# lightkurve/lightkurve

Hardware: NVIDIA B200
Metric: lombscargle_freqbins_x_cadences_per_s (higher is better)
Workload: dtype f32 spreading + FFT, f64 phase (nufft)

## Files before the change

### lightkurve_b200/csrc/nufft_v2.cuh

```cuda
#pragma once
#include "nufft_core.h"

namespace lkb {
namespace {

using nufft::V2_PB;
using nufft::V2_THREADS;
using nufft::V2_TILE;
constexpr int V2_LOG_TILE = 13;
static_assert((1 << V2_LOG_TILE) == V2_TILE, "tile size");
constexpr int V2_BC = 1 << V2_PB;
constexpr int V2_R = V2_TILE / (2 * V2_BC);
constexpr int V2_LSB = V2_BC + V2_BC / 16 + 1;
constexpr int V2R_P_MIN = V2_PB + 4 + 1, V2R_P_MAX = V2_PB + 13 + 1;

__host__ __device__ constexpr int v2_radix(int plog, int idx) {
  return (idx < plog / 4) ? 16 : ((idx == plog / 4 && (plog % 4)) ? (1 << (plog % 4)) : 0);
}
__host__ __device__ constexpr int v2_log2i(int r) { return r == 16 ? 4 : r == 8 ? 3 : r == 4 ? 2 : r == 2 ? 1 : 0; }
__device__ __forceinline__ int v2_skew(int a) { return a + (a >> 4); }
template <int nb>
__host__ __device__ constexpr int v2_in_off(int r) {
  return (nb % 16 == 0) ? r * (nb + nb / 16) : r * nb + ((r * nb) >> 4);
}

template <class CT>
__global__ void nufft2_tables_kernel(int pa, int pb, int ph, CT* __restrict__ tw_a, CT* __restrict__ tw_b,
                                     CT* __restrict__ t_hi, CT* __restrict__ t_lo) {
  const int la = nufft::v2_pass_table_len(pa), lb = nufft::v2_pass_table_len(pb), pl = nufft::v2_log2_lo(ph);
  const int nlo = 1 << pl, nhi = 1 << (ph - pl);
  int e = (int)(blockIdx.x * blockDim.x + threadIdx.x);
  int64_t num = 0, den = 1;
  CT* dst = nullptr;
  if (e < la) { nufft::v2_pass_table_entry(pa, e, &num, &den); dst = tw_a + e; }
  else if ((e -= la) < lb) { nufft::v2_pass_table_entry(pb, e, &num, &den); dst = tw_b + e; }
  else if ((e -= lb) < nhi) { num = e; den = nhi; dst = t_hi + e; }
  else if ((e -= nhi) < nlo) { num = e; den = (int64_t)1 << ph; dst = t_lo + e; }
  else return;
  double sn, cs;
  sincospi(2.0 * (double)num / (double)den, &sn, &cs);
  typedef typename nufft::CplxOf<CT>::real RT;
  *dst = nufft::CplxOf<CT>::mk((RT)cs, (RT)sn);
}

template <class RT>
__global__ void nufft2_weights_kernel(const double* __restrict__ t, int64_t N, double df, int64_t M, int w, double beta,
                                      RT* __restrict__ Wt) {
  const int64_t e = (int64_t)blockIdx.x * blockDim.x + threadIdx.x;
  if (e >= N * w) return;
  const int64_t n = e / w;
  const int q = (int)(e - n * w);
  const double x = df * t[n] * (double)M + (double)nufft::grid_shift(w);
  const double i0 = ceil(x - 0.5 * (double)w);
  const double z = (i0 + (double)q - x) * (2.0 / (double)w);
  const double s2 = 1.0 - z * z;
  Wt[e] = (s2 > 0.0) ? (RT)exp(beta * (sqrt(s2) - 1.0)) : (RT)0.0;
}

__device__ __forceinline__ int64_t v2_zcell_of(int64_t e, int ptc, int n1max) {
  const int64_t j = e & (((int64_t)1 << ptc) - 1), rest = e >> ptc;
  const int64_t n1 = rest % n1max, c = rest / n1max;
  return (n1 << V2_PB) + (c << ptc) + j;
}

template <int LCS>
__global__ void __launch_bounds__(256)
nufft2_spread_kernel(const int32_t* __restrict__ first_ge, const nufft::Cad* __restrict__ cad,
                     const float* __restrict__ Wt, const float* __restrict__ y, int64_t ystride, int B, int w, int p,
                     int ptc, int n1max, float2* __restrict__ G) {
  const int64_t cells = (int64_t)n1max << V2_PB;
  const int64_t e = (int64_t)blockIdx.x * blockDim.x + threadIdx.x;
  if (e >= cells) return;
  const int64_t M = (int64_t)1 << p, m = 2 * v2_zcell_of(e, ptc, n1max);
  const int lc0 = (int)blockIdx.y * LCS;
  const float* yr[LCS];
#pragma unroll
  for (int q = 0; q < LCS; ++q) {
    int b = lc0 + q;
    if (b > B - 1) b = B - 1;
    yr[q] = y + (int64_t)b * ystride;
  }
  float a0[LCS], a1[LCS];
#pragma unroll
  for (int q = 0; q < LCS; ++q) { a0[q] = 0.0f; a1[q] = 0.0f; }
  const int64_t L = nufft::table_len(M, w);
  for (int wrap = 0; wrap < 2; ++wrap) {
    const int64_t mm = m + (int64_t)wrap * M;
    if (mm + 1 >= L) break;
    int64_t lo_c = mm - w + 1, hi_c = mm + 2;
    if (lo_c < 0) lo_c = 0;
    if (hi_c > L - 1) hi_c = L - 1;
    const int32_t na = first_ge[lo_c], nb = first_ge[hi_c];
    for (int32_t n = na; n < nb; ++n) {
      const int tap = (int)(mm - (int64_t)cad[n].i0);
      const float* wr = Wt + (int64_t)n * w;
      const float w0 = (tap >= 0) ? wr[tap] : 0.0f;
      const float w1 = (tap + 1 < w) ? wr[tap + 1] : 0.0f;
#pragma unroll
      for (int q = 0; q < LCS; ++q) {
        const float v = yr[q][n];
        a0[q] = fmaf(w0, v, a0[q]);
        a1[q] = fmaf(w1, v, a1[q]);
      }
    }
  }
#pragma unroll
  for (int q = 0; q < LCS; ++q)
    if (lc0 + q < B) G[(int64_t)(lc0 + q) * cells + e] = make_float2(a0[q], a1[q]);
}

template <int PLOG, int LS, int IDX, int NS, class CT = float2>
__device__ __forceinline__ void v2_pass_t(CT* buf, const CT* __restrict__ tw, int nz = 1 << 30) {
  constexpr int R = v2_radix(PLOG, IDX);
  if constexpr (R != 0) {
    constexpr int LR = v2_log2i(R), NB = 16 / R, PNB = PLOG - LR, nb = 1 << PNB;
    constexpr bool WIDE = nb > V2_THREADS;
    static_assert(WIDE || (V2_THREADS % nb) == 0, "geometry");
    const int t = (int)threadIdx.x;
    CT u[NB][R];
    int base_in[NB];
#pragma unroll
    for (int q = 0; q < NB; ++q) {
      int line, i;
      if constexpr (WIDE) { line = 0; i = t + V2_THREADS * q; }
      else { line = (t >> PNB) + ((V2_THREADS * q) >> PNB); i = t & (nb - 1); }
      base_in[q] = line * LS + ((nb % 16 == 0) ? v2_skew(i) : i);
#pragma unroll
      for (int r = 0; r < R; ++r)
        u[q][r] = (IDX > 0 || r * nb < nz) ? buf[base_in[q] + v2_in_off<nb>(r)] : nufft::CplxOf<CT>::mk(0, 0);
    }
    __syncthreads();
#pragma unroll
    for (int q = 0; q < NB; ++q) {
      int line, i;
      if constexpr (WIDE) { line = 0; i = t + V2_THREADS * q; }
      else { line = (t >> PNB) + ((V2_THREADS * q) >> PNB); i = t & (nb - 1); }
      const int k = i & (NS - 1);
      if constexpr (NS > 1) {
#pragma unroll
        for (int r = 1; r < R; ++r) u[q][r] = nufft::cmul(u[q][r], tw[r * NS + k]);
      }
      nufft::SmallDft<R, CT>::run(u[q]);
      const int j = ((i - k) << LR) + k;
      const int base_out = line * LS + ((NS == 1) ? (j + i) : v2_skew(j));
#pragma unroll
      for (int r = 0; r < R; ++r) buf[base_out + ((NS == 1) ? r : r * (NS + NS / 16))] = u[q][r];
    }
    __syncthreads();
    v2_pass_t<PLOG, LS, IDX + 1, NS * R, CT>(buf, tw + ((IDX > 0) ? R * NS : 0));
  }
}

struct V2Count {
  const int* count;
  int base, cap;
};
__device__ __forceinline__ int v2_count(const V2Count nc, int grid_y) {
  if (!nc.count) return grid_y;
  const int n = *nc.count - nc.base;
  return n < 0 ? 0 : (n > nc.cap ? nc.cap : n);
}

template <int PA, class CT>
__device__ __forceinline__ void v2_cols_one(CT* buf, const CT* __restrict__ G, CT* __restrict__ T, int n1max,
                                            const CT* __restrict__ tw_a, const CT* __restrict__ t_hi,
                                            const CT* __restrict__ t_lo, const int64_t lc) {
  constexpr int A = 1 << PA, PTC = V2_LOG_TILE - PA, TC = 1 << PTC, LS = A + A / 16 + 1, C = V2_BC / TC;
  constexpr int JW = TC < 32 ? TC : 32, RW = V2_THREADS / JW, CG = TC / JW;
  constexpr int LJW = JW == 32 ? 5 : JW == 16 ? 4 : JW == 8 ? 3 : JW == 4 ? 2 : JW == 2 ? 1 : 0;
  static_assert((1 << LJW) == JW && RW % 16 == 0, "geometry");
  const int t = (int)threadIdx.x, c = (int)blockIdx.x;
  const int jl = t & (JW - 1), nl = t >> LJW;
  const int nvalid = n1max << PTC;
  const CT* Gp = G + (lc * C + c) * (int64_t)nvalid;
  const int s_base = jl * LS + v2_skew(nl), g_base = nl * TC + jl;
  constexpr int NB1 = A / v2_radix(PA, 0);
  const int nz = ((n1max + NB1 - 1) / NB1) * NB1;
#pragma unroll
  for (int u = 0; u < 16; ++u) {
    const int cg = u % CG, nbk = u / CG;
    if (nbk * RW < nz) {
      const int idx = g_base + nbk * RW * TC + cg * JW;
      buf[s_base + cg * JW * LS + nbk * (RW + RW / 16)] = (idx < nvalid) ? Gp[idx] : nufft::CplxOf<CT>::mk(0, 0);
    }
  }
  __syncthreads();
  v2_pass_t<PA, LS, 0, 1, CT>(buf, tw_a, nz);
  CT* Tp = T + (lc * C + c) * (int64_t)V2_TILE;
  const int ph = PA + V2_PB, pl = nufft::v2_log2_lo(ph);
  const unsigned Mmask = (1u << ph) - 1u, lmask = (1u << pl) - 1u;
#pragma unroll
  for (int u = 0; u < 16; ++u) {
    const int cg = u % CG, nbk = u / CG;
    const int k1 = nl + nbk * RW, n2 = c * TC + jl + cg * JW;
    const unsigned q = ((unsigned)n2 * (unsigned)k1) & Mmask;
    const CT wq = nufft::cmul(t_hi[q >> pl], t_lo[q & lmask]);
    Tp[g_base + nbk * RW * TC + cg * JW] = nufft::cmul(buf[s_base + cg * JW * LS + nbk * (RW + RW / 16)], wq);
  }
}
template <int PA, class CT = float2>
__global__ void __launch_bounds__(V2_THREADS, sizeof(CT) == 8 ? 2 : 1)
nufft2_cols_kernel(const CT* __restrict__ G, CT* __restrict__ T, int n1max, const CT* __restrict__ tw_a,
                   const CT* __restrict__ t_hi, const CT* __restrict__ t_lo) {
  LKB_DYN_SMEM(CT, buf);
  v2_cols_one<PA, CT>(buf, G, T, n1max, tw_a, t_hi, t_lo, (int64_t)blockIdx.y);
}
template <int PA>
__global__ void __launch_bounds__(V2_THREADS, 1)
nufft2_cols_list_kernel(const double2* __restrict__ G, double2* __restrict__ T, int n1max,
                        const double2* __restrict__ tw_a, const double2* __restrict__ t_hi,
                        const double2* __restrict__ t_lo, V2Count nc) {
  LKB_DYN_SMEM(double2, buf);
  const int64_t ntr = v2_count(nc, (int)gridDim.y);
  for (int64_t lc = blockIdx.y; lc < ntr; lc += gridDim.y) {
    __syncthreads();
    v2_cols_one<PA, double2>(buf, G, T, n1max, tw_a, t_hi, t_lo, lc);
  }
}

struct V2FTab {
  float4 d;
  float4 c;
};
struct V2Finish {
  const V2FTab* ftab;
  int64_t k0, F, k_lo;
  const float* ysum;
  float Nf;
  int normalization;
  float scale;
  float* power;
  unsigned* peak;
  const int* lcmap;
  int log2M;
};

__device__ __forceinline__ float v2_normalise(float pw, float Nf, int normalization, float scale) {
  if (normalization == LKB_LS_NORM_PSD_SCALE) return pw * scale;
  if (normalization == LKB_LS_NORM_AMPLITUDE) return sqrtf(pw * (4.0f / Nf));
  return pw;
}
__device__ __forceinline__ float v2_finish_pw(float2 g1, float2 g2, const V2FTab tb, float ysum, int64_t, int) {
  const float ex = 0.5f * (g1.x + g2.x), ey = 0.5f * (g1.y - g2.y);
  const float ox = 0.5f * (g1.y + g2.y), oy = 0.5f * (g2.x - g1.x);
  const float yc = ex * tb.d.x - ey * tb.d.y + ox * tb.d.z - oy * tb.d.w - ysum * tb.c.x;
  const float ys = ex * tb.d.y + ey * tb.d.x + ox * tb.d.w + oy * tb.d.z - ysum * tb.c.y;
  return yc * yc * tb.c.z + ys * ys * tb.c.w;
}
__device__ __forceinline__ float v2_finish_pw(double2 g1, double2 g2, const V2FTab tb, float ysum, int64_t kk, int log2M) {
  const double ex = 0.5 * (g1.x + g2.x), ey = 0.5 * (g1.y - g2.y);
  const double ox = 0.5 * (g1.y + g2.y), oy = 0.5 * (g2.x - g1.x);
  double sw, cw;
  sincospi(ldexp((double)kk, 1 - log2M), &sw, &cw);
  const double gx = ex + cw * ox - sw * oy, gy = ey + cw * oy + sw * ox;
  const double yc = gx * (double)tb.d.x - gy * (double)tb.d.y - (double)ysum * (double)tb.c.x;
  const double ys = gx * (double)tb.d.y + gy * (double)tb.d.x - (double)ysum * (double)tb.c.y;
  return (float)(yc * yc * (double)tb.c.z + ys * ys * (double)tb.c.w);
}

template <int PA, int MODE, class CT>
__device__ __forceinline__ void v2_rows_one(CT* buf, const CT* __restrict__ T, const CT* __restrict__ tw_b,
                                            const V2Finish& fa, CT* __restrict__ Zout, int nk2_keep, const int64_t lc,
                                            const int lc_base, const int g) {
  constexpr int A = 1 << PA, PTC = V2_LOG_TILE - PA, TC = 1 << PTC, R = V2_R, LS = V2_LSB, Bc = V2_BC;
  const int t = (int)threadIdx.x;
  const bool last = g == (A / (2 * R)) - 1;
  const int64_t Mh = (int64_t)1 << (PA + V2_PB);
  auto slot_k1 = [&](int s) -> int {
    const int h = s >> 3, r = s & (R - 1);
    if (h == 0) return 1 + g * R + r;
    if (last && r == 0) return 0;
    return A - (g + 1) * R + r;
  };
  const CT* Tp = T + lc * Mh;
#pragma unroll
  for (int u = 0; u < 16; ++u) {
    const int e = t + V2_THREADS * u;
    const int j = e & (TC - 1), r = (e >> PTC) & (R - 1), h = (e >> (PTC + 3)) & 1, c = e >> (PTC + 4);
    const int s = h * R + r;
    buf[s * LS + v2_skew((c << PTC) + j)] = Tp[(((c << PA) + slot_k1(s)) << PTC) + j];
  }
  __syncthreads();
  v2_pass_t<V2_PB, LS, 0, 1, CT>(buf, tw_b);
  const int s = t & (2 * R - 1), h = s >> 3, r = s & (R - 1), k1 = slot_k1(s);
  if (MODE == 2) {
    const int keep = nk2_keep < Bc / 2 ? nk2_keep : Bc / 2;
    for (int q = t >> 4; q < 2 * keep; q += V2_THREADS / 16) {
      const int k2 = q < keep ? q : Bc - 2 * keep + q;
      Zout[lc * Mh + k1 + ((int64_t)k2 << PA)] = buf[s * LS + v2_skew(k2)];
    }
  } else {
  int ps = (1 - h) * R + (R - 1 - r);
  bool row0 = false;
  if (last && h == 0 && r == R - 1) ps = s;
  if (last && h == 1 && r == 0) { ps = s; row0 = true; }
  int64_t nK2 = ((fa.k0 + fa.F - 1) >> PA) + 1;
  if (nK2 > Bc) nK2 = Bc;
  const int64_t lcd = fa.lcmap ? (int64_t)fa.lcmap[lc_base + lc] : lc;
  const float ys0 = fa.ysum[lcd];
  float* prow = fa.power + lcd * fa.F;
  const int64_t jbase = (int64_t)k1 - fa.k0;
  float pmax = 0.0f;
  constexpr int KSTEP = V2_THREADS / 16, UB = 4;
  for (int k2b = t >> 4; k2b < (int)nK2; k2b += KSTEP * UB) {
    V2FTab tb[UB];
    int64_t jj[UB];
    bool valid[UB];
#pragma unroll
    for (int u = 0; u < UB; ++u) {
      const int k2 = k2b + KSTEP * u;
      jj[u] = jbase + ((int64_t)k2 << PA);
      valid[u] = k2 < (int)nK2 && jj[u] >= fa.k_lo && jj[u] < fa.F;
      if (valid[u]) tb[u] = fa.ftab[jj[u]];
    }
#pragma unroll
    for (int u = 0; u < UB; ++u) {
      if (!valid[u]) continue;
      const int k2 = k2b + KSTEP * u;
      const int pi = row0 ? ((Bc - k2) & (Bc - 1)) : (Bc - 1 - k2);
      const CT g1 = buf[s * LS + v2_skew(k2)], g2 = buf[ps * LS + v2_skew(pi)];
      const float pw = v2_finish_pw(g1, g2, tb[u], ys0, fa.k0 + jj[u], fa.log2M);
      pmax = fmaxf(pmax, pw);
      prow[jj[u]] = v2_normalise(pw, fa.Nf, fa.normalization, fa.scale);
    }
  }
  if (fa.peak) {
#pragma unroll
    for (int o = 16; o > 0; o >>= 1) pmax = fmaxf(pmax, __shfl_xor_sync(0xffffffffu, pmax, o));
    if ((t & 31) == 0 && pmax > 0.0f) atomicMax(fa.peak + lcd, __float_as_uint(pmax));
  }
  }
}

template <int PA, int MODE, class CT = float2>
__global__ void __launch_bounds__(V2_THREADS, sizeof(CT) == 8 ? 2 : 1)
nufft2_rows_kernel(const CT* __restrict__ T, const CT* __restrict__ tw_b, V2Finish fa, CT* __restrict__ Zout,
                   int nk2_keep) {
  LKB_DYN_SMEM(CT, buf);
  v2_rows_one<PA, MODE, CT>(buf, T, tw_b, fa, Zout, nk2_keep, (int64_t)blockIdx.y, 0, (int)blockIdx.x);
}
template <int PA>
__global__ void __launch_bounds__(V2_THREADS, 1)
nufft2_rows_list_kernel(const double2* __restrict__ T, const double2* __restrict__ tw_b, V2Finish fa, V2Count nc) {
  LKB_DYN_SMEM(double2, buf);
  const int64_t ntr = v2_count(nc, (int)gridDim.y);
  for (int64_t lc = blockIdx.y; lc < ntr; lc += gridDim.y) {
    __syncthreads();
    v2_rows_one<PA, 1, double2>(buf, T, tw_b, fa, nullptr, 0, lc, nc.base, (int)blockIdx.x);
  }
}

__global__ void nufft2_flag_kernel(const unsigned* __restrict__ peak, const float* __restrict__ absmax, int B, float Nf,
                                   float ratio, int* __restrict__ count, int* __restrict__ list, int* __restrict__ total) {
  const int b = (int)(blockIdx.x * blockDim.x + threadIdx.x);
  bool f = false;
  if (b < B) {
    const float amp = sqrtf(__uint_as_float(peak[b]) * (4.0f / Nf));
    f = absmax[b] > ratio * amp;
  }
  const unsigned bal = __ballot_sync(0xffffffffu, f);
  if (bal) {
    int base = 0;
    if ((threadIdx.x & 31) == 0) {
      base = atomicAdd(count, __popc(bal));
      if (total) atomicAdd(total, __popc(bal));
    }
    base = __shfl_sync(0xffffffffu, base, 0);
    if (f) list[base + __popc(bal & ((1u << (threadIdx.x & 31)) - 1u))] = b;
  }
}

__global__ void __launch_bounds__(256)
nufft2_spread_list_kernel(const int32_t* __restrict__ first_ge, const nufft::Cad* __restrict__ cad,
                          const double* __restrict__ Wt, const float* __restrict__ y, int64_t ystride,
                          const int* __restrict__ list, int w, int p, int ptc, int n1max, double2* __restrict__ G,
                          V2Count nc) {
  const int64_t cells = (int64_t)n1max << V2_PB;
  const int64_t e = (int64_t)blockIdx.x * blockDim.x + threadIdx.x;
  if (e >= cells) return;
  const int64_t M = (int64_t)1 << p, m = 2 * v2_zcell_of(e, ptc, n1max);
  const int ntr = v2_count(nc, (int)gridDim.y);
  for (int i = (int)blockIdx.y; i < ntr; i += (int)gridDim.y) {
  const float* yr = y + (int64_t)list[nc.base + i] * ystride;
  double a0 = 0.0, a1 = 0.0;
  const int64_t L = nufft::table_len(M, w);
  for (int wrap = 0; wrap < 2; ++wrap) {
    const int64_t mm = m + (int64_t)wrap * M;
    if (mm + 1 >= L) break;
    int64_t lo_c = mm - w + 1, hi_c = mm + 2;
    if (lo_c < 0) lo_c = 0;
    if (hi_c > L - 1) hi_c = L - 1;
    const int32_t na = first_ge[lo_c], nb = first_ge[hi_c];
    for (int32_t n = na; n < nb; ++n) {
      const int tap = (int)(mm - (int64_t)cad[n].i0);
      const double* wr = Wt + (int64_t)n * w;
      const double w0 = (tap >= 0) ? wr[tap] : 0.0, w1 = (tap + 1 < w) ? wr[tap + 1] : 0.0;
      const double v = (double)yr[n];
      a0 = fma(w0, v, a0);
      a1 = fma(w1, v, a1);
    }
  }
  G[(int64_t)i * cells + e] = make_double2(a0, a1);
  }
}

inline unsigned v2_blocks_for(int64_t n, int per) { return (unsigned)((n + per - 1) / per); }

template <class CT>
struct V2TablesT {
  const CT *tw_a, *tw_b, *t_hi, *t_lo;
};
typedef V2TablesT<float2> V2Tables;
typedef V2TablesT<double2> V2TablesD;
template <class CT>
inline int v2_tables(int p, int slot, cudaStream_t st, V2TablesT<CT>* out) {
  const int ph = p - 1, pa = ph - V2_PB, pl = nufft::v2_log2_lo(ph);
  const int la = nufft::v2_pass_table_len(pa), lb = nufft::v2_pass_table_len(V2_PB), nhi = 1 << (ph - pl), nlo = 1 << pl;
  CT* base = nullptr;
  LKB_TRY(ws_get_t<CT>(slot, (size_t)(la + lb + nhi + nlo + 4), &base));
  CT *tw_a = base, *tw_b = base + la, *t_hi = tw_b + lb, *t_lo = t_hi + nhi;
  LKB_LAUNCH(v2_blocks_for(la + lb + nhi + nlo, 256), 256, st, nufft2_tables_kernel<CT>)(pa, V2_PB, ph, tw_a, tw_b, t_hi, t_lo);
  LKB_LAUNCH_CHECK();
  out->tw_a = tw_a; out->tw_b = tw_b; out->t_hi = t_hi; out->t_lo = t_lo;
  return LKB_OK;
}
inline int v2_n1max(int p, int64_t i0_last, int w) {
  const int64_t M = (int64_t)1 << p, A = (M / 2) >> V2_PB;
  const int64_t reach = i0_last + w + 1;
  if (reach >= M) return (int)A;
  const int64_t n = ((reach + 1) / 2 + V2_BC - 1) >> V2_PB;
  return (int)(n < 1 ? 1 : (n > A ? A : n));
}
inline bool v2_supported(int p) { return p >= V2R_P_MIN && p <= V2R_P_MAX; }

template <int PA, class CT>
int v2_cols_pa(const CT* G, CT* T, int n1max, int B, const V2TablesT<CT>& tb, cudaStream_t st, V2Count nc) {
  constexpr int A = 1 << PA, TC = V2_TILE / A;
  const size_t smem = (size_t)TC * (A + A / 16 + 1) * sizeof(CT);
  const dim3 grid((unsigned)(V2_BC / TC), (unsigned)B);
  if constexpr (sizeof(CT) == 16) {
    if (nc.count) {
      LKB_CUDA_CHECK(cudaFuncSetAttribute(nufft2_cols_list_kernel<PA>, cudaFuncAttributeMaxDynamicSharedMemorySize, (int)smem));
      LKB_LAUNCH_SMEM(grid, V2_THREADS, smem, st, nufft2_cols_list_kernel<PA>)(G, T, n1max, tb.tw_a, tb.t_hi, tb.t_lo, nc);
      LKB_LAUNCH_CHECK();
      return LKB_OK;
    }
  }
  LKB_CUDA_CHECK(cudaFuncSetAttribute(nufft2_cols_kernel<PA, CT>, cudaFuncAttributeMaxDynamicSharedMemorySize, (int)smem));
  LKB_LAUNCH_SMEM(grid, V2_THREADS, smem, st, nufft2_cols_kernel<PA, CT>)(G, T, n1max, tb.tw_a, tb.t_hi, tb.t_lo);
  LKB_LAUNCH_CHECK();
  return LKB_OK;
}
template <int PA, class CT>
int v2_rows_pa(const CT* T, int B, const V2TablesT<CT>& tb, const V2Finish* fa, CT* Zout, int nk2_keep, cudaStream_t st,
               V2Count nc) {
  const size_t smem = (size_t)(2 * V2_R) * V2_LSB * sizeof(CT);
  const dim3 grid((unsigned)((1 << PA) / (2 * V2_R)), (unsigned)B);
  if constexpr (sizeof(CT) == 16) {
    if (nc.count && fa) {
      LKB_CUDA_CHECK(cudaFuncSetAttribute(nufft2_rows_list_kernel<PA>, cudaFuncAttributeMaxDynamicSharedMemorySize, (int)smem));
      LKB_LAUNCH_SMEM(grid, V2_THREADS, smem, st, nufft2_rows_list_kernel<PA>)(T, tb.tw_b, *fa, nc);
      LKB_LAUNCH_CHECK();
      return LKB_OK;
    }
  }
  LKB_CUDA_CHECK(cudaFuncSetAttribute(nufft2_rows_kernel<PA, 1, CT>, cudaFuncAttributeMaxDynamicSharedMemorySize, (int)smem));
  LKB_CUDA_CHECK(cudaFuncSetAttribute(nufft2_rows_kernel<PA, 2, CT>, cudaFuncAttributeMaxDynamicSharedMemorySize, (int)smem));
  if (fa) LKB_LAUNCH_SMEM(grid, V2_THREADS, smem, st, nufft2_rows_kernel<PA, 1, CT>)(T, tb.tw_b, *fa, nullptr, 0);
  else LKB_LAUNCH_SMEM(grid, V2_THREADS, smem, st, nufft2_rows_kernel<PA, 2, CT>)(T, tb.tw_b, V2Finish(), Zout, nk2_keep);
  LKB_LAUNCH_CHECK();
  return LKB_OK;
}
#define V2_DISPATCH_PA(pa, CALL)                                                                       \
  switch (pa) {                                                                                         \
    case 4: return CALL(4); case 5: return CALL(5); case 6: return CALL(6); case 7: return CALL(7);      \
    case 8: return CALL(8); case 9: return CALL(9); case 10: return CALL(10); case 11: return CALL(11);  \
    case 12: return CALL(12); case 13: return CALL(13);                                                  \
    default: set_error("NUFFT v2: fine grid of 2^%d cells out of range", (pa) + V2_PB + 1); return LKB_E_UNSUPPORTED; \
  }
template <class CT>
inline int v2_cols(const CT* G, CT* T, int p, int n1max, int B, const V2TablesT<CT>& tb, cudaStream_t st,
                   V2Count nc = V2Count{nullptr, 0, 0}) {
#define V2_CALL(PA) v2_cols_pa<PA, CT>(G, T, n1max, B, tb, st, nc)
  V2_DISPATCH_PA(p - 1 - V2_PB, V2_CALL)
#undef V2_CALL
}
template <class CT>
inline int v2_rows(const CT* T, int p, int B, const V2TablesT<CT>& tb, const V2Finish* fa, CT* Zout, int nk2_keep,
                   cudaStream_t st, V2Count nc = V2Count{nullptr, 0, 0}) {
#define V2_CALL(PA) v2_rows_pa<PA, CT>(T, B, tb, fa, Zout, nk2_keep, st, nc)
  V2_DISPATCH_PA(p - 1 - V2_PB, V2_CALL)
#undef V2_CALL
}

}
}
```

### lightkurve_b200/csrc/ptx.cuh

```cuda
#pragma once
#include <stdint.h>
#include <cuda.h>

namespace lkb {
namespace ptx {

__device__ __forceinline__ uint32_t smem_u32(const void* p) {
  return static_cast<uint32_t>(__cvta_generic_to_shared(p));
}

__device__ __forceinline__ void mbar_init(uint64_t* bar, uint32_t count) {
  asm volatile("mbarrier.init.shared::cta.b64 [%0], %1;" ::"r"(smem_u32(bar)), "r"(count) : "memory");
}
__device__ __forceinline__ void mbar_fence_init() {
  asm volatile("fence.mbarrier_init.release.cluster;" ::: "memory");
}
__device__ __forceinline__ void mbar_arrive_expect_tx(uint64_t* bar, uint32_t bytes) {
  asm volatile("mbarrier.arrive.expect_tx.shared::cta.b64 _, [%0], %1;" ::"r"(smem_u32(bar)), "r"(bytes)
               : "memory");
}
__device__ __forceinline__ void mbar_arrive(uint64_t* bar) {
  asm volatile("mbarrier.arrive.shared::cta.b64 _, [%0];" ::"r"(smem_u32(bar)) : "memory");
}
__device__ __forceinline__ bool mbar_try_wait(uint64_t* bar, uint32_t parity) {
  uint32_t ok;
  asm volatile(
      "{\n\t.reg .pred p;\n\t"
      "mbarrier.try_wait.parity.shared::cta.b64 p, [%1], %2;\n\t"
      "selp.u32 %0, 1, 0, p;\n\t}"
      : "=r"(ok)
      : "r"(smem_u32(bar)), "r"(parity)
      : "memory");
  return ok != 0;
}
__device__ __forceinline__ bool mbar_try_wait_hint(uint64_t* bar, uint32_t parity, uint32_t hint_ns) {
  uint32_t ok;
  asm volatile(
      "{\n\t.reg .pred p;\n\t"
      "mbarrier.try_wait.parity.shared::cta.b64 p, [%1], %2, %3;\n\t"
      "selp.u32 %0, 1, 0, p;\n\t}"
      : "=r"(ok)
      : "r"(smem_u32(bar)), "r"(parity), "r"(hint_ns)
      : "memory");
  return ok != 0;
}
__device__ __forceinline__ void mbar_wait_park(uint64_t* bar, uint32_t parity, uint32_t hint_ns) {
  while (!mbar_try_wait_hint(bar, parity, hint_ns)) {
  }
}
__device__ __forceinline__ void mbar_wait(uint64_t* bar, uint32_t parity) {
  while (!mbar_try_wait(bar, parity)) {
  }
}
__device__ __forceinline__ void mbar_wait_sleep(uint64_t* bar, uint32_t parity, uint32_t ns) {
  while (!mbar_try_wait(bar, parity)) {
    if (ns) __nanosleep(ns);
  }
}

__device__ __forceinline__ void fence_proxy_async_smem() {
  asm volatile("fence.proxy.async.shared::cta;" ::: "memory");
}
__device__ __forceinline__ void bulk_g2s(void* dst_smem, const void* src_gmem, uint32_t bytes, uint64_t* bar) {
  asm volatile(
      "cp.async.bulk.shared::cluster.global.mbarrier::complete_tx::bytes [%0], [%1], %2, [%3];" ::"r"(
          smem_u32(dst_smem)),
      "l"(src_gmem), "r"(bytes), "r"(smem_u32(bar))
      : "memory");
}
__device__ __forceinline__ void tma_load_2d(void* dst_smem, const CUtensorMap* map, int32_t c0, int32_t c1,
                                            uint64_t* bar) {
  asm volatile(
      "cp.async.bulk.tensor.2d.shared::cluster.global.tile.mbarrier::complete_tx::bytes [%0], [%1, {%3, %4}], [%2];" ::
          "r"(smem_u32(dst_smem)),
      "l"(map), "r"(smem_u32(bar)), "r"(c0), "r"(c1)
      : "memory");
}
__device__ __forceinline__ void prefetch_tensormap(const CUtensorMap* map) {
  asm volatile("prefetch.tensormap [%0];" ::"l"(map) : "memory");
}

__device__ __forceinline__ void tmem_alloc(uint32_t* dst_smem, uint32_t ncols) {
  asm volatile("tcgen05.alloc.cta_group::1.sync.aligned.shared::cta.b32 [%0], %1;" ::"r"(smem_u32(dst_smem)),
               "r"(ncols)
               : "memory");
}
__device__ __forceinline__ void tmem_relinquish() {
  asm volatile("tcgen05.relinquish_alloc_permit.cta_group::1.sync.aligned;" ::: "memory");
}
__device__ __forceinline__ void tmem_dealloc(uint32_t taddr, uint32_t ncols) {
  asm volatile("tcgen05.dealloc.cta_group::1.sync.aligned.b32 %0, %1;" ::"r"(taddr), "r"(ncols) : "memory");
}
__device__ __forceinline__ void tc_fence_before() {
  asm volatile("tcgen05.fence::before_thread_sync;" ::: "memory");
}
__device__ __forceinline__ void tc_fence_after() {
  asm volatile("tcgen05.fence::after_thread_sync;" ::: "memory");
}
__device__ __forceinline__ void umma_f16_ss(uint32_t tmem_d, uint64_t desc_a, uint64_t desc_b, uint32_t idesc,
                                            uint32_t accumulate) {
  asm volatile(
      "{\n\t.reg .pred p;\n\t"
      "setp.ne.b32 p, %4, 0;\n\t"
      "tcgen05.mma.cta_group::1.kind::f16 [%0], %1, %2, %3, p;\n\t}" ::"r"(tmem_d),
      "l"(desc_a), "l"(desc_b), "r"(idesc), "r"(accumulate)
      : "memory");
}
__device__ __forceinline__ void umma_commit(uint64_t* bar) {
  asm volatile("tcgen05.commit.cta_group::1.mbarrier::arrive::one.shared::cluster.b64 [%0];" ::"r"(smem_u32(bar))
               : "memory");
}
__device__ __forceinline__ void tmem_ld_32x32b_x32(uint32_t taddr, uint32_t* v) {
  asm volatile(
      "tcgen05.ld.sync.aligned.32x32b.x32.b32 "
      "{%0, %1, %2, %3, %4, %5, %6, %7, %8, %9, %10, %11, %12, %13, %14, %15, "
      "%16, %17, %18, %19, %20, %21, %22, %23, %24, %25, %26, %27, %28, %29, %30, %31}, [%32];"
      : "=r"(v[0]), "=r"(v[1]), "=r"(v[2]), "=r"(v[3]), "=r"(v[4]), "=r"(v[5]), "=r"(v[6]), "=r"(v[7]),
        "=r"(v[8]), "=r"(v[9]), "=r"(v[10]), "=r"(v[11]), "=r"(v[12]), "=r"(v[13]), "=r"(v[14]), "=r"(v[15]),
        "=r"(v[16]), "=r"(v[17]), "=r"(v[18]), "=r"(v[19]), "=r"(v[20]), "=r"(v[21]), "=r"(v[22]), "=r"(v[23]),
        "=r"(v[24]), "=r"(v[25]), "=r"(v[26]), "=r"(v[27]), "=r"(v[28]), "=r"(v[29]), "=r"(v[30]), "=r"(v[31])
      : "r"(taddr)
      : "memory");
}
__device__ __forceinline__ void tmem_ld_32x32b_x16(uint32_t taddr, uint32_t* v) {
  asm volatile(
      "tcgen05.ld.sync.aligned.32x32b.x16.b32 "
      "{%0, %1, %2, %3, %4, %5, %6, %7, %8, %9, %10, %11, %12, %13, %14, %15}, [%16];"
      : "=r"(v[0]), "=r"(v[1]), "=r"(v[2]), "=r"(v[3]), "=r"(v[4]), "=r"(v[5]), "=r"(v[6]), "=r"(v[7]),
        "=r"(v[8]), "=r"(v[9]), "=r"(v[10]), "=r"(v[11]), "=r"(v[12]), "=r"(v[13]), "=r"(v[14]), "=r"(v[15])
      : "r"(taddr)
      : "memory");
}
__device__ __forceinline__ void tmem_ld_wait() { asm volatile("tcgen05.wait::ld.sync.aligned;" ::: "memory"); }


__device__ __forceinline__ uint32_t cluster_ctarank() {
  uint32_t r;
  asm volatile("mov.u32 %0, %%cluster_ctarank;" : "=r"(r));
  return r;
}
__device__ __forceinline__ void cluster_sync() {
  asm volatile("barrier.cluster.arrive.release.aligned;\n\tbarrier.cluster.wait.acquire.aligned;" ::: "memory");
}
__device__ __forceinline__ uint32_t leader_addr(const void* p) {
  uint32_t r;
  asm volatile("mapa.shared::cluster.u32 %0, %1, %2;" : "=r"(r) : "r"(smem_u32(p)), "r"(0));
  return r;
}
__device__ __forceinline__ void mbar_arrive_cluster(uint32_t cluster_addr) {
  asm volatile("mbarrier.arrive.release.cluster.shared::cluster.b64 _, [%0];" ::"r"(cluster_addr) : "memory");
}
__device__ __forceinline__ bool mbar_try_wait_cluster(uint64_t* bar, uint32_t parity) {
  uint32_t ok;
  asm volatile(
      "{\n\t.reg .pred p;\n\t"
      "mbarrier.try_wait.parity.acquire.cluster.shared::cta.b64 p, [%1], %2;\n\t"
      "selp.u32 %0, 1, 0, p;\n\t}"
      : "=r"(ok)
      : "r"(smem_u32(bar)), "r"(parity)
      : "memory");
  return ok != 0;
}
__device__ __forceinline__ void mbar_wait_cluster_sleep(uint64_t* bar, uint32_t parity, uint32_t ns) {
  while (!mbar_try_wait_cluster(bar, parity)) __nanosleep(ns);
}
__device__ __forceinline__ void tma_load_2d_2sm(void* dst_smem, const CUtensorMap* map, int32_t c0, int32_t c1,
                                                uint32_t leader_bar) {
  asm volatile(
      "cp.async.bulk.tensor.2d.cta_group::2.shared::cluster.global.mbarrier::complete_tx::bytes"
      " [%0], [%1, {%3, %4}], [%2];" ::"r"(smem_u32(dst_smem)),
      "l"(map), "r"(leader_bar), "r"(c0), "r"(c1)
      : "memory");
}
__device__ __forceinline__ void tmem_alloc_2cta(uint32_t* dst_smem, uint32_t ncols) {
  asm volatile("tcgen05.alloc.cta_group::2.sync.aligned.shared::cta.b32 [%0], %1;" ::"r"(smem_u32(dst_smem)),
               "r"(ncols)
               : "memory");
}
__device__ __forceinline__ void tmem_relinquish_2cta() {
  asm volatile("tcgen05.relinquish_alloc_permit.cta_group::2.sync.aligned;" ::: "memory");
}
__device__ __forceinline__ void tmem_dealloc_2cta(uint32_t taddr, uint32_t ncols) {
  asm volatile("tcgen05.dealloc.cta_group::2.sync.aligned.b32 %0, %1;" ::"r"(taddr), "r"(ncols) : "memory");
}
__device__ __forceinline__ void umma_f16_ss_2cta(uint32_t tmem_d, uint64_t desc_a, uint64_t desc_b, uint32_t idesc,
                                                 uint32_t accumulate) {
  asm volatile(
      "{\n\t.reg .pred p;\n\t"
      "setp.ne.b32 p, %4, 0;\n\t"
      "tcgen05.mma.cta_group::2.kind::f16 [%0], %1, %2, %3, p;\n\t}" ::"r"(tmem_d),
      "l"(desc_a), "l"(desc_b), "r"(idesc), "r"(accumulate)
      : "memory");
}
__device__ __forceinline__ void umma_commit_2cta(uint64_t* bar) {
  const uint16_t mask = 3;
  asm volatile("tcgen05.commit.cta_group::2.mbarrier::arrive::one.shared::cluster.multicast::cluster.b64 [%0], %1;" ::
                   "r"(smem_u32(bar)),
               "h"(mask)
               : "memory");
}

}
}
```

Baseline: 1685000 billion.

## Pipeline NUFFT row FFT through persistent warp-specialised cp.async triple-buffer ring

Replaces the float32 rows kernel with a persistent kernel sized to the SM count. Each CTA runs two independent 256-thread groups that share a 3-slot shared-memory ring. Tiles are prefetched with cp.async and tracked by mbarriers, so global loads of the next tile overlap the FFT and finish work on the current one, with named barriers per group. The load and compute phases are split into separate functions, the finish-loop unroll drops from 4 to 2, and a host emulation of the new PTX primitives is added. Risks include lower occupancy from one large CTA per SM, extra mbarrier overhead, and fragile ring synchronisation.

Result: faster. 1905000 billion, median of 6 (+13.1%).

```diff
diff --git a/lightkurve_b200/csrc/nufft_v2.cuh b/lightkurve_b200/csrc/nufft_v2.cuh
--- a/lightkurve_b200/csrc/nufft_v2.cuh
+++ b/lightkurve_b200/csrc/nufft_v2.cuh
@@ -1,5 +1,6 @@
 #pragma once
 #include "nufft_core.h"
+#include "ptx.cuh"
 
 namespace lkb {
 namespace {
@@ -109,14 +110,31 @@
     if (lc0 + q < B) G[(int64_t)(lc0 + q) * cells + e] = make_float2(a0[q], a1[q]);
 }
 
-template <int PLOG, int LS, int IDX, int NS, class CT = float2>
-__device__ __forceinline__ void v2_pass_t(CT* buf, const CT* __restrict__ tw, int nz = 1 << 30) {
+struct V2Cta {
+  __device__ __forceinline__ int tid() const { return (int)threadIdx.x; }
+  __device__ __forceinline__ void sync() const { __syncthreads(); }
+  template <class CT>
+  __device__ __forceinline__ void put(CT* dst, const CT* src, bool ok) const {
+    *dst = ok ? *src : nufft::CplxOf<CT>::mk(0, 0);
+  }
+};
+struct V2Half {
+  __device__ __forceinline__ static int group() { return ptx::tid_x() / V2_THREADS; }
+  __device__ __forceinline__ int tid() const { return ptx::tid_x() & (V2_THREADS - 1); }
+  __device__ __forceinline__ void sync() const { ptx::bar_sync_named(1 + group(), V2_THREADS); }
+  __device__ __forceinline__ void put(float2* dst, const float2* src, bool ok) const {
+    ptx::cp_async_8(dst, src, ok ? 8u : 0u);
+  }
+};
+
+template <int PLOG, int LS, int IDX, int NS, class CT, class Grp>
+__device__ __forceinline__ void v2_pass_t(CT* buf, const CT* __restrict__ tw, const Grp gp, int nz = 1 << 30) {
   constexpr int R = v2_radix(PLOG, IDX);
   if constexpr (R != 0) {
     constexpr int LR = v2_log2i(R), NB = 16 / R, PNB = PLOG - LR, nb = 1 << PNB;
     constexpr bool WIDE = nb > V2_THREADS;
     static_assert(WIDE || (V2_THREADS % nb) == 0, "geometry");
-    const int t = (int)threadIdx.x;
+    const int t = gp.tid();
     CT u[NB][R];
     int base_in[NB];
 #pragma unroll
@@ -129,7 +147,7 @@
       for (int r = 0; r < R; ++r)
         u[q][r] = (IDX > 0 || r * nb < nz) ? buf[base_in[q] + v2_in_off<nb>(r)] : nufft::CplxOf<CT>::mk(0, 0);
     }
-    __syncthreads();
+    gp.sync();
 #pragma unroll
     for (int q = 0; q < NB; ++q) {
       int line, i;
@@ -146,8 +164,8 @@
 #pragma unroll
       for (int r = 0; r < R; ++r) buf[base_out + ((NS == 1) ? r : r * (NS + NS / 16))] = u[q][r];
     }
-    __syncthreads();
-    v2_pass_t<PLOG, LS, IDX + 1, NS * R, CT>(buf, tw + ((IDX > 0) ? R * NS : 0));
+    gp.sync();
+    v2_pass_t<PLOG, LS, IDX + 1, NS * R, CT>(buf, tw + ((IDX > 0) ? R * NS : 0), gp);
   }
 }
 
@@ -161,49 +179,64 @@
   return n < 0 ? 0 : (n > nc.cap ? nc.cap : n);
 }
 
-template <int PA, class CT>
-__device__ __forceinline__ void v2_cols_one(CT* buf, const CT* __restrict__ G, CT* __restrict__ T, int n1max,
-                                            const CT* __restrict__ tw_a, const CT* __restrict__ t_hi,
-                                            const CT* __restrict__ t_lo, const int64_t lc) {
-  constexpr int A = 1 << PA, PTC = V2_LOG_TILE - PA, TC = 1 << PTC, LS = A + A / 16 + 1, C = V2_BC / TC;
-  constexpr int JW = TC < 32 ? TC : 32, RW = V2_THREADS / JW, CG = TC / JW;
-  constexpr int LJW = JW == 32 ? 5 : JW == 16 ? 4 : JW == 8 ? 3 : JW == 4 ? 2 : JW == 2 ? 1 : 0;
+template <int PA>
+struct V2Cols {
+  static constexpr int A = 1 << PA, PTC = V2_LOG_TILE - PA, TC = 1 << PTC, LS = A + A / 16 + 1, C = V2_BC / TC;
+  static constexpr int ELEMS = TC * LS;
+  static constexpr int JW = TC < 32 ? TC : 32, RW = V2_THREADS / JW, CG = TC / JW;
+  static constexpr int LJW = JW == 32 ? 5 : JW == 16 ? 4 : JW == 8 ? 3 : JW == 4 ? 2 : JW == 2 ? 1 : 0;
   static_assert((1 << LJW) == JW && RW % 16 == 0, "geometry");
-  const int t = (int)threadIdx.x, c = (int)blockIdx.x;
-  const int jl = t & (JW - 1), nl = t >> LJW;
-  const int nvalid = n1max << PTC;
-  const CT* Gp = G + (lc * C + c) * (int64_t)nvalid;
-  const int s_base = jl * LS + v2_skew(nl), g_base = nl * TC + jl;
-  constexpr int NB1 = A / v2_radix(PA, 0);
-  const int nz = ((n1max + NB1 - 1) / NB1) * NB1;
+  static constexpr int NB1 = A / v2_radix(PA, 0);
+  __device__ __forceinline__ static int nz(int n1max) { return ((n1max + NB1 - 1) / NB1) * NB1; }
+};
+template <int PA, class CT, class Grp>
+__device__ __forceinline__ void v2_cols_load(CT* buf, const CT* __restrict__ G, int n1max, const int64_t lc, const int c,
+                                             const Grp gp) {
+  using Q = V2Cols<PA>;
+  const int t = gp.tid();
+  const int jl = t & (Q::JW - 1), nl = t >> Q::LJW;
+  const int nvalid = n1max << Q::PTC, nz = Q::nz(n1max);
+  const CT* Gp = G + (lc * Q::C + c) * (int64_t)nvalid;
+  const int s_base = jl * Q::LS + v2_skew(nl), g_base = nl * Q::TC + jl;
 #pragma unroll
   for (int u = 0; u < 16; ++u) {
-    const int cg = u % CG, nbk = u / CG;
-    if (nbk * RW < nz) {
-      const int idx = g_base + nbk * RW * TC + cg * JW;
-      buf[s_base + cg * JW * LS + nbk * (RW + RW / 16)] = (idx < nvalid) ? Gp[idx] : nufft::CplxOf<CT>::mk(0, 0);
-    }
-  }
-  __syncthreads();
-  v2_pass_t<PA, LS, 0, 1, CT>(buf, tw_a, nz);
-  CT* Tp = T + (lc * C + c) * (int64_t)V2_TILE;
+    const int cg = u % Q::CG, nbk = u / Q::CG;
+    if (nbk * Q::RW < nz) {
+      const int idx = g_base + nbk * Q::RW * Q::TC + cg * Q::JW;
+      gp.put(buf + s_base + cg * Q::JW * Q::LS + nbk * (Q::RW + Q::RW / 16), Gp + (idx < nvalid ? idx : 0), idx < nvalid);
+    }
+  }
+}
+template <int PA, class CT, class Grp>
+__device__ __forceinline__ void v2_cols_one(CT* buf, CT* __restrict__ T, int n1max, const CT* __restrict__ tw_a,
+                                            const CT* __restrict__ t_hi, const CT* __restrict__ t_lo, const int64_t lc,
+                                            const int c, const Grp gp) {
+  using Q = V2Cols<PA>;
+  const int t = gp.tid();
+  const int jl = t & (Q::JW - 1), nl = t >> Q::LJW;
+  const int s_base = jl * Q::LS + v2_skew(nl), g_base = nl * Q::TC + jl;
+  v2_pass_t<PA, Q::LS, 0, 1, CT>(buf, tw_a, gp, Q::nz(n1max));
+  CT* Tp = T + (lc * Q::C + c) * (int64_t)V2_TILE;
   const int ph = PA + V2_PB, pl = nufft::v2_log2_lo(ph);
   const unsigned Mmask = (1u << ph) - 1u, lmask = (1u << pl) - 1u;
 #pragma unroll
   for (int u = 0; u < 16; ++u) {
-    const int cg = u % CG, nbk = u / CG;
-    const int k1 = nl + nbk * RW, n2 = c * TC + jl + cg * JW;
+    const int cg = u % Q::CG, nbk = u / Q::CG;
+    const int k1 = nl + nbk * Q::RW, n2 = c * Q::TC + jl + cg * Q::JW;
     const unsigned q = ((unsigned)n2 * (unsigned)k1) & Mmask;
     const CT wq = nufft::cmul(t_hi[q >> pl], t_lo[q & lmask]);
-    Tp[g_base + nbk * RW * TC + cg * JW] = nufft::cmul(buf[s_base + cg * JW * LS + nbk * (RW + RW / 16)], wq);
-  }
-}
-template <int PA, class CT = float2>
-__global__ void __launch_bounds__(V2_THREADS, sizeof(CT) == 8 ? 2 : 1)
-nufft2_cols_kernel(const CT* __restrict__ G, CT* __restrict__ T, int n1max, const CT* __restrict__ tw_a,
-                   const CT* __restrict__ t_hi, const CT* __restrict__ t_lo) {
-  LKB_DYN_SMEM(CT, buf);
-  v2_cols_one<PA, CT>(buf, G, T, n1max, tw_a, t_hi, t_lo, (int64_t)blockIdx.y);
+    Tp[g_base + nbk * Q::RW * Q::TC + cg * Q::JW] =
+        nufft::cmul(buf[s_base + cg * Q::JW * Q::LS + nbk * (Q::RW + Q::RW / 16)], wq);
+  }
+}
+template <int PA>
+__global__ void __launch_bounds__(V2_THREADS, 2)
+nufft2_cols_kernel(const float2* __restrict__ G, float2* __restrict__ T, int n1max, const float2* __restrict__ tw_a,
+                   const float2* __restrict__ t_hi, const float2* __restrict__ t_lo) {
+  LKB_DYN_SMEM(float2, buf);
+  v2_cols_load<PA>(buf, G, n1max, (int64_t)blockIdx.y, (int)blockIdx.x, V2Cta());
+  __syncthreads();
+  v2_cols_one<PA>(buf, T, n1max, tw_a, t_hi, t_lo, (int64_t)blockIdx.y, (int)blockIdx.x, V2Cta());
 }
 template <int PA>
 __global__ void __launch_bounds__(V2_THREADS, 1)
@@ -214,10 +247,34 @@
   const int64_t ntr = v2_count(nc, (int)gridDim.y);
   for (int64_t lc = blockIdx.y; lc < ntr; lc += gridDim.y) {
     __syncthreads();
-    v2_cols_one<PA, double2>(buf, G, T, n1max, tw_a, t_hi, t_lo, lc);
-  }
-}
-
+    v2_cols_load<PA>(buf, G, n1max, lc, (int)blockIdx.x, V2Cta());
+    __syncthreads();
+    v2_cols_one<PA>(buf, T, n1max, tw_a, t_hi, t_lo, lc, (int)blockIdx.x, V2Cta());
+  }
+}
+
+template <class Load, class Body>
+__device__ __forceinline__ void v2_ring(float2* smem, const int elems, const int ntiles, Load load, Body body) {
+  uint64_t* bar = reinterpret_cast<uint64_t*>(smem + 3 * elems);
+  const V2Half gp{};
+  if (threadIdx.x < 6) ptx::mbar_init(bar + threadIdx.x, V2_THREADS);
+  __syncthreads();
+  const int b = (int)blockIdx.x, nb = (int)gridDim.x;
+  auto fetch = [&](int j) {
+    if (b + j * nb < ntiles) {
+      load(smem + (j % 3) * elems, b + j * nb, gp);
+      ptx::cp_async_mbar_arrive_noinc(bar + j % 6);
+    }
+  };
+  for (int j = V2Half::group(); j < 3; j += 2) fetch(j);
+  for (int j = V2Half::group(); b + j * nb < ntiles; j += 2) {
+    ptx::mbar_wait(bar + j % 6, (uint32_t)(j / 6) & 1u);
+    body(smem + (j % 3) * elems, b + j * nb, gp);
+    gp.sync();
+    fetch(j + 3);
+  }
+  ptx::cp_async_wait_all();
+}
 struct V2FTab {
   float4 d;
   float4 c;
@@ -258,31 +315,38 @@
   return (float)(yc * yc * (double)tb.c.z + ys * ys * (double)tb.c.w);
 }
 
-template <int PA, int MODE, class CT>
-__device__ __forceinline__ void v2_rows_one(CT* buf, const CT* __restrict__ T, const CT* __restrict__ tw_b,
-                                            const V2Finish& fa, CT* __restrict__ Zout, int nk2_keep, const int64_t lc,
-                                            const int lc_base, const int g) {
-  constexpr int A = 1 << PA, PTC = V2_LOG_TILE - PA, TC = 1 << PTC, R = V2_R, LS = V2_LSB, Bc = V2_BC;
-  const int t = (int)threadIdx.x;
-  const bool last = g == (A / (2 * R)) - 1;
-  const int64_t Mh = (int64_t)1 << (PA + V2_PB);
-  auto slot_k1 = [&](int s) -> int {
-    const int h = s >> 3, r = s & (R - 1);
-    if (h == 0) return 1 + g * R + r;
-    if (last && r == 0) return 0;
-    return A - (g + 1) * R + r;
-  };
-  const CT* Tp = T + lc * Mh;
+template <int PA>
+__device__ __forceinline__ int v2_slot_k1(int s, int g) {
+  constexpr int A = 1 << PA, R = V2_R;
+  const int h = s >> 3, r = s & (R - 1);
+  if (h == 0) return 1 + g * R + r;
+  if (g == (A / (2 * R)) - 1 && r == 0) return 0;
+  return A - (g + 1) * R + r;
+}
+template <int PA, class CT, class Grp>
+__device__ __forceinline__ void v2_rows_load(CT* buf, const CT* __restrict__ T, const int64_t lc, const int g,
+                                             const Grp gp) {
+  constexpr int PTC = V2_LOG_TILE - PA, TC = 1 << PTC, R = V2_R, LS = V2_LSB;
+  const int t = gp.tid();
+  const CT* Tp = T + (lc << (PA + V2_PB));
 #pragma unroll
   for (int u = 0; u < 16; ++u) {
     const int e = t + V2_THREADS * u;
     const int j = e & (TC - 1), r = (e >> PTC) & (R - 1), h = (e >> (PTC + 3)) & 1, c = e >> (PTC + 4);
     const int s = h * R + r;
-    buf[s * LS + v2_skew((c << PTC) + j)] = Tp[(((c << PA) + slot_k1(s)) << PTC) + j];
-  }
-  __syncthreads();
-  v2_pass_t<V2_PB, LS, 0, 1, CT>(buf, tw_b);
-  const int s = t & (2 * R - 1), h = s >> 3, r = s & (R - 1), k1 = slot_k1(s);
+    gp.put(buf + s * LS + v2_skew((c << PTC) + j), Tp + ((((c << PA) + v2_slot_k1<PA>(s, g)) << PTC) + j), true);
+  }
+}
+template <int PA, int MODE, class CT, class Grp>
+__device__ __forceinline__ void v2_rows_one(CT* buf, const CT* __restrict__ tw_b, const V2Finish& fa,
+                                            CT* __restrict__ Zout, int nk2_keep, const int64_t lc, const int lc_base,
+                                            const int g, const Grp gp) {
+  constexpr int A = 1 << PA, R = V2_R, LS = V2_LSB, Bc = V2_BC;
+  const int t = gp.tid();
+  const bool last = g == (A / (2 * R)) - 1;
+  const int64_t Mh = (int64_t)1 << (PA + V2_PB);
+  v2_pass_t<V2_PB, LS, 0, 1, CT>(buf, tw_b, gp);
+  const int s = t & (2 * R - 1), h = s >> 3, r = s & (R - 1), k1 = v2_slot_k1<PA>(s, g);
   if (MODE == 2) {
     const int keep = nk2_keep < Bc / 2 ? nk2_keep : Bc / 2;
     for (int q = t >> 4; q < 2 * keep; q += V2_THREADS / 16) {
@@ -301,7 +365,7 @@
   float* prow = fa.power + lcd * fa.F;
   const int64_t jbase = (int64_t)k1 - fa.k0;
   float pmax = 0.0f;
-  constexpr int KSTEP = V2_THREADS / 16, UB = 4;
+  constexpr int KSTEP = V2_THREADS / 16, UB = 2;
   for (int k2b = t >> 4; k2b < (int)nK2; k2b += KSTEP * UB) {
     V2FTab tb[UB];
     int64_t jj[UB];
@@ -332,13 +396,6 @@
   }
 }
 
-template <int PA, int MODE, class CT = float2>
-__global__ void __launch_bounds__(V2_THREADS, sizeof(CT) == 8 ? 2 : 1)
-nufft2_rows_kernel(const CT* __restrict__ T, const CT* __restrict__ tw_b, V2Finish fa, CT* __restrict__ Zout,
-                   int nk2_keep) {
-  LKB_DYN_SMEM(CT, buf);
-  v2_rows_one<PA, MODE, CT>(buf, T, tw_b, fa, Zout, nk2_keep, (int64_t)blockIdx.y, 0, (int)blockIdx.x);
-}
 template <int PA>
 __global__ void __launch_bounds__(V2_THREADS, 1)
 nufft2_rows_list_kernel(const double2* __restrict__ T, const double2* __restrict__ tw_b, V2Finish fa, V2Count nc) {
@@ -346,8 +403,22 @@
   const int64_t ntr = v2_count(nc, (int)gridDim.y);
   for (int64_t lc = blockIdx.y; lc < ntr; lc += gridDim.y) {
     __syncthreads();
-    v2_rows_one<PA, 1, double2>(buf, T, tw_b, fa, nullptr, 0, lc, nc.base, (int)blockIdx.x);
-  }
+    v2_rows_load<PA>(buf, T, lc, (int)blockIdx.x, V2Cta());
+    __syncthreads();
+    v2_rows_one<PA, 1>(buf, tw_b, fa, (double2*)nullptr, 0, lc, nc.base, (int)blockIdx.x, V2Cta());
+  }
+}
+template <int PA, int MODE>
+__global__ void __launch_bounds__(2 * V2_THREADS, 1)
+nufft2_rows_ring_kernel(const float2* __restrict__ T, const float2* __restrict__ tw_b, V2Finish fa,
+                        float2* __restrict__ Zout, int nk2_keep, int B) {
+  constexpr int NG = (1 << PA) / (2 * V2_R);
+  LKB_DYN_SMEM(float2, smem);
+  v2_ring(smem, 2 * V2_R * V2_LSB, B * NG,
+          [&](float2* buf, int tile, const V2Half gp) { v2_rows_load<PA>(buf, T, tile / NG, tile % NG, gp); },
+          [&](float2* buf, int tile, const V2Half gp) {
+            v2_rows_one<PA, MODE>(buf, tw_b, fa, Zout, nk2_keep, tile / NG, 0, tile % NG, gp);
+          });
 }
 
 __global__ void nufft2_flag_kernel(const unsigned* __restrict__ peak, const float* __restrict__ absmax, int B, float Nf,
@@ -433,41 +504,48 @@
 }
 inline bool v2_supported(int p) { return p >= V2R_P_MIN && p <= V2R_P_MAX; }
 
+inline size_t v2_ring_smem(int elems) { return 3 * (size_t)elems * sizeof(float2) + 6 * sizeof(uint64_t); }
+inline unsigned v2_ring_ctas(int64_t ntiles) {
+#if defined(LKB_CUDA_EMU)
+  int64_t n = 2;
+#else
+  int64_t n = sm_count();
+#endif
+  if (const char* e = getenv("LKB_NUFFT_RING_CTAS")) n = std::max(1, atoi(e));
+  return (unsigned)std::max<int64_t>(1, std::min<int64_t>(n, ntiles));
+}
+
 template <int PA, class CT>
 int v2_cols_pa(const CT* G, CT* T, int n1max, int B, const V2TablesT<CT>& tb, cudaStream_t st, V2Count nc) {
-  constexpr int A = 1 << PA, TC = V2_TILE / A;
-  const size_t smem = (size_t)TC * (A + A / 16 + 1) * sizeof(CT);
-  const dim3 grid((unsigned)(V2_BC / TC), (unsigned)B);
+  using Q = V2Cols<PA>;
+  const size_t smem = (size_t)Q::ELEMS * sizeof(CT);
+  const dim3 grid((unsigned)Q::C, (unsigned)B);
   if constexpr (sizeof(CT) == 16) {
-    if (nc.count) {
-      LKB_CUDA_CHECK(cudaFuncSetAttribute(nufft2_cols_list_kernel<PA>, cudaFuncAttributeMaxDynamicSharedMemorySize, (int)smem));
-      LKB_LAUNCH_SMEM(grid, V2_THREADS, smem, st, nufft2_cols_list_kernel<PA>)(G, T, n1max, tb.tw_a, tb.t_hi, tb.t_lo, nc);
-      LKB_LAUNCH_CHECK();
-      return LKB_OK;
-    }
-  }
-  LKB_CUDA_CHECK(cudaFuncSetAttribute(nufft2_cols_kernel<PA, CT>, cudaFuncAttributeMaxDynamicSharedMemorySize, (int)smem));
-  LKB_LAUNCH_SMEM(grid, V2_THREADS, smem, st, nufft2_cols_kernel<PA, CT>)(G, T, n1max, tb.tw_a, tb.t_hi, tb.t_lo);
+    LKB_CUDA_CHECK(cudaFuncSetAttribute(nufft2_cols_list_kernel<PA>, cudaFuncAttributeMaxDynamicSharedMemorySize, (int)smem));
+    LKB_LAUNCH_SMEM(grid, V2_THREADS, smem, st, nufft2_cols_list_kernel<PA>)(G, T, n1max, tb.tw_a, tb.t_hi, tb.t_lo, nc);
+  } else {
+    LKB_CUDA_CHECK(cudaFuncSetAttribute(nufft2_cols_kernel<PA>, cudaFuncAttributeMaxDynamicSharedMemorySize, (int)smem));
+    LKB_LAUNCH_SMEM(grid, V2_THREADS, smem, st, nufft2_cols_kernel<PA>)(G, T, n1max, tb.tw_a, tb.t_hi, tb.t_lo);
+  }
   LKB_LAUNCH_CHECK();
   return LKB_OK;
 }
 template <int PA, class CT>
 int v2_rows_pa(const CT* T, int B, const V2TablesT<CT>& tb, const V2Finish* fa, CT* Zout, int nk2_keep, cudaStream_t st,
                V2Count nc) {
-  const size_t smem = (size_t)(2 * V2_R) * V2_LSB * sizeof(CT);
-  const dim3 grid((unsigned)((1 << PA) / (2 * V2_R)), (unsigned)B);
+  constexpr int NG = (1 << PA) / (2 * V2_R);
   if constexpr (sizeof(CT) == 16) {
-    if (nc.count && fa) {
-      LKB_CUDA_CHECK(cudaFuncSetAttribute(nufft2_rows_list_kernel<PA>, cudaFuncAttributeMaxDynamicSharedMemorySize, (int)smem));
-      LKB_LAUNCH_SMEM(grid, V2_THREADS, smem, st, nufft2_rows_list_kernel<PA>)(T, tb.tw_b, *fa, nc);
-      LKB_LAUNCH_CHECK();
-      return LKB_OK;
-    }
-  }
-  LKB_CUDA_CHECK(cudaFuncSetAttribute(nufft2_rows_kernel<PA, 1, CT>, cudaFuncAttributeMaxDynamicSharedMemorySize, (int)smem));
-  LKB_CUDA_CHECK(cudaFuncSetAttribute(nufft2_rows_kernel<PA, 2, CT>, cudaFuncAttributeMaxDynamicSharedMemorySize, (int)smem));
-  if (fa) LKB_LAUNCH_SMEM(grid, V2_THREADS, smem, st, nufft2_rows_kernel<PA, 1, CT>)(T, tb.tw_b, *fa, nullptr, 0);
-  else LKB_LAUNCH_SMEM(grid, V2_THREADS, smem, st, nufft2_rows_kernel<PA, 2, CT>)(T, tb.tw_b, V2Finish(), Zout, nk2_keep);
+    const size_t smem = (size_t)(2 * V2_R) * V2_LSB * sizeof(CT);
+    LKB_CUDA_CHECK(cudaFuncSetAttribute(nufft2_rows_list_kernel<PA>, cudaFuncAttributeMaxDynamicSharedMemorySize, (int)smem));
+    LKB_LAUNCH_SMEM(dim3((unsigned)NG, (unsigned)B), V2_THREADS, smem, st, nufft2_rows_list_kernel<PA>)(T, tb.tw_b, *fa, nc);
+  } else {
+    const size_t smem = v2_ring_smem(2 * V2_R * V2_LSB);
+    const unsigned grid = v2_ring_ctas((int64_t)B * NG);
+    LKB_CUDA_CHECK(cudaFuncSetAttribute(nufft2_rows_ring_kernel<PA, 1>, cudaFuncAttributeMaxDynamicSharedMemorySize, (int)smem));
+    LKB_CUDA_CHECK(cudaFuncSetAttribute(nufft2_rows_ring_kernel<PA, 2>, cudaFuncAttributeMaxDynamicSharedMemorySize, (int)smem));
+    if (fa) LKB_LAUNCH_SMEM(grid, 2 * V2_THREADS, smem, st, nufft2_rows_ring_kernel<PA, 1>)(T, tb.tw_b, *fa, nullptr, 0, B);
+    else LKB_LAUNCH_SMEM(grid, 2 * V2_THREADS, smem, st, nufft2_rows_ring_kernel<PA, 2>)(T, tb.tw_b, V2Finish(), Zout, nk2_keep, B);
+  }
   LKB_LAUNCH_CHECK();
   return LKB_OK;
 }
diff --git a/lightkurve_b200/csrc/ptx.cuh b/lightkurve_b200/csrc/ptx.cuh
--- a/lightkurve_b200/csrc/ptx.cuh
+++ b/lightkurve_b200/csrc/ptx.cuh
@@ -1,4 +1,5 @@
 #pragma once
+#if !defined(LKB_CUDA_EMU)
 #include <stdint.h>
 #include <cuda.h>
 
@@ -57,6 +58,25 @@
     if (ns) __nanosleep(ns);
   }
 }
+
+__device__ __forceinline__ int tid_x() {
+  int t;
+  asm volatile("mov.u32 %0, %%tid.x;" : "=r"(t));
+  return t;
+}
+
+__device__ __forceinline__ void bar_sync_named(int id, int nthreads) {
+  asm volatile("bar.sync %0, %1;" ::"r"(id), "r"(nthreads) : "memory");
+}
+__device__ __forceinline__ void cp_async_8(void* dst_smem, const void* src_gmem, uint32_t src_bytes) {
+  asm volatile("cp.async.ca.shared.global [%0], [%1], 8, %2;" ::"r"(smem_u32(dst_smem)), "l"(src_gmem), "r"(src_bytes)
+               : "memory");
+}
+__device__ __forceinline__ void cp_async_mbar_arrive_noinc(uint64_t* bar) {
+  asm volatile("cp.async.mbarrier.arrive.noinc.shared::cta.b64 [%0];" ::"r"(smem_u32(bar)) : "memory");
+}
+
+__device__ __forceinline__ void cp_async_wait_all() { asm volatile("cp.async.wait_all;" ::: "memory"); }
 
 __device__ __forceinline__ void fence_proxy_async_smem() {
   asm volatile("fence.proxy.async.shared::cta;" ::: "memory");
@@ -202,3 +222,64 @@
 
 }
 }
+
+#else
+#include <stdint.h>
+#include <string.h>
+#include <condition_variable>
+#include <mutex>
+
+namespace lkb {
+namespace ptx {
+struct EmuSync {
+  std::mutex m;
+  std::condition_variable cv;
+  int arrived[16] = {};
+  long generation[16] = {};
+};
+inline EmuSync& emu_sync() {
+  static EmuSync s;
+  return s;
+}
+inline int tid_x() { return (int)threadIdx.x; }
+inline void bar_sync_named(int id, int nthreads) {
+  EmuSync& e = emu_sync();
+  std::unique_lock<std::mutex> lk(e.m);
+  const long gen = e.generation[id];
+  if (++e.arrived[id] == nthreads) {
+    e.arrived[id] = 0;
+    ++e.generation[id];
+    e.cv.notify_all();
+    return;
+  }
+  e.cv.wait(lk, [&] { return gen != e.generation[id]; });
+}
+inline void mbar_init(uint64_t* bar, uint32_t count) {
+  std::lock_guard<std::mutex> lk(emu_sync().m);
+  *bar = (uint64_t)count | ((uint64_t)count << 32);
+}
+inline void mbar_arrive(uint64_t* bar) {
+  EmuSync& e = emu_sync();
+  std::lock_guard<std::mutex> lk(e.m);
+  const uint64_t count = *bar & 0xffffffffull, phase = *bar >> 63, pending = ((*bar >> 32) & 0x7fffffffull) - 1;
+  if (pending == 0) {
+    *bar = count | (count << 32) | ((phase ^ 1ull) << 63);
+    e.cv.notify_all();
+  } else {
+    *bar = count | (pending << 32) | (phase << 63);
+  }
+}
+inline void mbar_wait(uint64_t* bar, uint32_t parity) {
+  EmuSync& e = emu_sync();
+  std::unique_lock<std::mutex> lk(e.m);
+  e.cv.wait(lk, [&] { return (uint32_t)(*bar >> 63) != (parity & 1u); });
+}
+inline void cp_async_8(void* dst_smem, const void* src_gmem, uint32_t src_bytes) {
+  memset(dst_smem, 0, 8);
+  if (src_bytes) memcpy(dst_smem, src_gmem, src_bytes);
+}
+inline void cp_async_mbar_arrive_noinc(uint64_t* bar) { mbar_arrive(bar); }
+inline void cp_async_wait_all() {}
+}
+}
+#endif
```
